# jinlong17/DA-Detect

Hardware: AMD Instinct MI355X
Metric: train images/sec, DA-Faster-RCNN R-50 Cityscapes->Foggy (higher is better)
Workload: dtype f32

## Files before the change

### da_detect_amd/_C.py

```python
import contextlib
import os
import ctypes
import time

import torch

from . import _lib
from . import amax as _amax
from ._lib import ConvDesc

CL = torch.channels_last

NMS_TIE_RULE = 0

PROFILER = None
_KNAME_CACHE = {}


class KernelProfiler(object):

    def __init__(self, pool=0, only=None):
        self.only = only
        self._pool = []
        for _ in range(pool):
# ... 716 lines not shown
        return g_out, g_scaled
    so = ss = None
    if g_out is not None and _amax.slot_of(_amax.carry(g_out, g)) is None:
        so = _amax.new_slot(g.device)
    if scale is not None or _amax.slot_of(_amax.carry(g_scaled, g)) is None:
        ss = _amax.new_slot(g.device)
    _lib.call("dadet_relu_bn_backward_m", _p(g), _p(yy), _p(scale), _p(g_out), _p(g_scaled), rows, C,
              ctypes.c_void_p(so[0]) if so else None, ctypes.c_void_p(ss[0]) if ss else None, _stream())
    if so:
        _amax.attach(g_out, so)
    if ss:
        _amax.attach(g_scaled, ss)
    return g_out, g_scaled


def colsum(g, out=None, accumulate=False, cols=None):
    _dev(g, "g")
    g = _nhwc(g) if g.dim() == 4 else g.contiguous()
    ld = g.shape[1]
    C = ld if cols is None else int(cols)
    rows = g.numel() // ld
    if out is None:
        out = torch.empty(C, dtype=torch.float32, device=g.device)
        accumulate = False
    assert out.numel() == C and out.is_contiguous() and out.dtype == torch.float32
    nbytes = ctypes.c_size_t(0)
    _lib.call("dadet_colsum_workspace_bytes", rows, C, ctypes.byref(nbytes))
    ws = _workspace(nbytes.value, g.device)
    _lib.call("dadet_colsum_ld", _p(g), ld, _p(out), rows, C, 1 if accumulate else 0, _p(ws), ctypes.c_size_t(ws.numel()),
              _stream())
# ... 39 lines not shown
    _dev(x, "x")
    x = _nhwc(x)
    R, C, h, w = x.shape
    y = torch.empty((R, C), dtype=torch.float32, device=x.device)
    _lib.call("dadet_avgpool_forward", _p(x), _p(y), R, h * w, C, _stream())
    return _amax.carry(y, x)


def avgpool_backward(gy, h, w):
    _dev(gy, "gy")
    gy = gy.contiguous()
    R, C = gy.shape
    gx = torch.empty((R, C, h, w), dtype=torch.float32, device=gy.device, memory_format=CL)
    _lib.call("dadet_avgpool_backward", _p(gy), _p(gx), R, h * w, C, _stream())
    return _amax.carry(gx, gy)


def nchw3_to_nhwc4(x):
    _dev(x, "x")
    x = x.contiguous()
    N, C, H, W = x.shape
    assert C == 3
    y = torch.empty((N, 4, H, W), dtype=torch.float32, device=x.device, memory_format=CL)
    _lib.call("dadet_nchw3_to_nhwc4", _p(x), _p(y), N, H, W, _stream())
    if _mode4():
        _amax.ptr(x)
        _amax.carry(y, x)
    return y


# ... 675 lines not shown
```

### da_detect_amd/_lib.py

```python
import ctypes
import os
from ctypes import POINTER, c_char_p, c_float, c_int, c_int64, c_size_t, c_uint64, c_void_p

_HERE = os.path.dirname(os.path.abspath(__file__))
LIB_PATH = os.environ.get("DADET_LIB") or os.path.join(_HERE, "libdadet_hip.so")
_lib = None
DEFAULT_GEMM_MODE = "4"


class ConvDesc(ctypes.Structure):

    _fields_ = [(n, c_int) for n in (
        "N", "H", "W", "Cin", "Cout", "KH", "KW", "stride", "pad", "Ho", "Wo", "OutH", "OutW",
        "out_spatial_stride", "relu_mode")]


class ConvPlanInfo(ctypes.Structure):

    _fields_ = [(n, c_int) for n in (
        "family", "variant", "tiles_m", "tiles_n", "ksplit", "splits", "rows_per_split", "sk_dp_tiles", "sk_tiles", "sk_units",
        "sk_iters", "sk_max_parts", "big_splits", "big_body", "launches", "grid", "needs_counters")] + [
        ("workspace_bytes", c_size_t), ("name", ctypes.c_char * 64)]


# ... 116 lines not shown
    "dadet_sample_anchors": [_P, _P, c_int, c_int, c_int, c_uint64, c_int64, _P, _P, _P, _P, _P],
    "dadet_topk_sorted": [_P, c_int, c_int, c_int64, c_int, _P, _P, _P],
    "dadet_topk_sorted_rows_workspace_bytes": [c_int, c_int, POINTER(c_size_t)],
    "dadet_topk_sorted_rows": [POINTER(TopkRow), c_int, _P, c_size_t, _P],
    "dadet_rpn_anchor_targets": [_P, _P, c_int, _P, c_int, c_float, c_float, _P, _P, _P, _P],
    "dadet_box_match_encode": [_P, c_int, _P, _P, c_int, c_float, c_float, c_float, c_float, c_float, c_float, _P, _P,
                               _P, _P],
    "dadet_roi_pool_forward": [_P, _P, _P, _P, c_int, c_int, c_int, c_int, c_int, c_int, c_int, c_float, _P],
    "dadet_roi_pool_backward": [_P, _P, _P, _P, c_int, c_int, c_int, c_int, c_int, c_int, c_int, _P],
    "dadet_deform_psroi_pool_forward": [_P, _P, _P, _P, _P, c_int, c_int, c_int, c_int, c_int, c_int, c_float,
                                        c_int, c_int, c_int, c_int, c_int, c_float, c_int, _P],
    "dadet_deform_psroi_pool_backward": [_P, _P, _P, _P, _P, _P, _P, c_int, c_int, c_int, c_int, c_int, c_int,
                                         c_float, c_int, c_int, c_int, c_int, c_int, c_float, c_int, _P],
    "dadet_relu_bn_backward": [_P, _P, _P, _P, _P, c_int64, c_int, _P],
    "dadet_relu_bn_backward_m": [_P, _P, _P, _P, _P, c_int64, c_int, _P, _P, _P],
    "dadet_colsum_workspace_bytes": [c_int64, c_int, POINTER(c_size_t)],
    "dadet_colsum": [_P, _P, c_int64, c_int, _P, c_size_t, _P],
    "dadet_colsum_ld": [_P, c_int, _P, c_int64, c_int, c_int, _P, c_size_t, _P],
    "dadet_channel_affine": [_P, _P, _P, _P, c_int64, c_int, c_int, _P],
    "dadet_maxpool3x3s2_forward": [_P, _P, c_int, c_int, c_int, c_int, c_int, c_int, _P],
    "dadet_maxpool3x3s2_relu_backward": [_P, _P, _P, _P, c_int, c_int, c_int, c_int, c_int, c_int, _P, _P],
    "dadet_avgpool_forward": [_P, _P, c_int, c_int, c_int, _P],
    "dadet_avgpool_backward": [_P, _P, c_int, c_int, c_int, _P],
    "dadet_nchw3_to_nhwc4": [_P, _P, c_int, c_int, c_int, _P],
    "dadet_rpn_decode_clip": [_P, _P, _P, c_int, c_float, c_float, c_float, c_float, c_float, c_float, c_float, _P, _P],
    "dadet_da_img_head_loss_forward": [_P, _P, _P, _P, _P, _P, c_int, c_int, c_int, _P],
    "dadet_da_img_head_loss_backward": [_P, _P, _P, _P, _P, _P, _P, _P, _P, c_int, c_int, c_int, _P],
    "dadet_da_img_head_loss_backward_g": [_P, _P, _P, _P, _P, _P, _P, c_float, c_float, _P, _P, _P, _P, c_int, c_int, c_int,
                                          _P],
    "dadet_da_img_head_loss_backward_gm": [_P, _P, _P, _P, _P, _P, _P, c_float, c_float, _P, _P, _P, _P, c_int, c_int, c_int,
                                          _P, _P, _P],
    "dadet_da_ins_tail_forward": [_P, _P, _P, _P, _P, _P, _P, c_int, c_int, c_int, c_int, c_int, _P],
    "dadet_da_ins_tail_backward": [_P, _P, _P, _P, _P, _P, c_float, _P, _P, _P, _P, c_int, c_int, c_int, c_int, c_int, _P],
    "dadet_da_ins_tail_forward_n": [_P, _P, _P, _P, _P, _P, _P, c_int, c_int, POINTER(c_int), c_int, c_int, c_int, _P],
    "dadet_da_ins_tail_backward_n": [_P, _P, _P, _P, _P, _P, c_float, _P, _P, _P, _P, c_int, c_int, POINTER(c_int), c_int,
                                     c_int, c_int, _P],
    "dadet_da_ins_dropout_rows": [_P, _P, _P, c_int64, c_int, _P],
    "dadet_da_ins_merge": [_P, _P, _P, _P, _P, _P, c_int64, c_int, _P],
# ... 45 lines not shown
```

### da_detect_amd/csrc/elementwise.hip

```cpp
#include "box_match.h"
#include "conv_common.h"
#include <float.h>

namespace dadet {

static inline int stream_blocks(int64_t work_items, int threads) {
  int64_t b = ceil_div64(work_items, threads);
  if (b > kMaxStreamBlocks) b = kMaxStreamBlocks;
  if (b < 1) b = 1;
  return (int)b;
}

__global__ void relu_bn_backward_kernel(const float4* __restrict__ g, const float4* __restrict__ y,
                                        const float4* __restrict__ scale, float4* __restrict__ g_out,
                                        float4* __restrict__ g_scaled, int64_t total4, int C4,
                                        unsigned* __restrict__ amax_out, unsigned* __restrict__ amax_scaled) {
  float mo = 0.f, ms = 0.f;
  for (int64_t i = (int64_t)blockIdx.x * blockDim.x + threadIdx.x; i < total4;
       i += (int64_t)gridDim.x * blockDim.x) {
    const float4 gv = g[i];
    float4 r = gv;
    if (y) {
      const float4 yv = y[i];
      r.x = yv.x > 0.f ? gv.x : 0.f;
// ... 3 lines not shown
    }
    if (g_out) g_out[i] = r;
    mo = fmaxf(fmaxf(mo, fmaxf(fabsf(r.x), fabsf(r.y))), fmaxf(fabsf(r.z), fabsf(r.w)));
    if (g_scaled) {
      float4 s = r;
      if (scale) {
        const float4 sc = scale[i % C4];
        s.x *= sc.x; s.y *= sc.y; s.z *= sc.z; s.w *= sc.w;
      }
      g_scaled[i] = s;
      ms = fmaxf(fmaxf(ms, fmaxf(fabsf(s.x), fabsf(s.y))), fmaxf(fabsf(s.z), fabsf(s.w)));
    }
  }
  if (amax_out) amax_publish(amax_out, mo);
  if (amax_scaled) amax_publish(amax_scaled, ms);
}

__global__ __launch_bounds__(256) void colsum_partial_kernel(const float* __restrict__ g,
                                                             float* __restrict__ partial, int64_t rows,
                                                             int C, int64_t rows_per_split, int cb, int ld) {
  __shared__ float red[256];
  const int lanes = 256 / cb;
  const int cl = threadIdx.x % cb, rl = threadIdx.x / cb;
  const int col = blockIdx.x * cb + cl;
  const int64_t r0 = (int64_t)blockIdx.y * rows_per_split;
  int64_t r1 = r0 + rows_per_split;
  if (r1 > rows) r1 = rows;
  float acc = 0.f;
  if (col < C)
    for (int64_t r = r0 + rl; r < r1; r += lanes) acc += g[r * ld + col];
// ... 143 lines not shown
}
__global__ void avgpool_bwd_kernel(const float4* __restrict__ gy, float4* __restrict__ gx, int R, int HW,
                                   int C4) {
  const int64_t total = (int64_t)R * HW * C4;
  const float inv = (float)HW;
  for (int64_t i = (int64_t)blockIdx.x * blockDim.x + threadIdx.x; i < total;
       i += (int64_t)gridDim.x * blockDim.x) {
    const int c = (int)(i % C4);
    const int64_t r = i / ((int64_t)HW * C4);
    float4 g = gy[r * C4 + c];
    g.x /= inv; g.y /= inv; g.z /= inv; g.w /= inv;
    gx[i] = g;
  }
}

__global__ void nchw3_to_nhwc4_kernel(const float* __restrict__ x, float4* __restrict__ y, int N,
                                      int64_t HW) {
  const int64_t total = (int64_t)N * HW;
  for (int64_t i = (int64_t)blockIdx.x * blockDim.x + threadIdx.x; i < total;
       i += (int64_t)gridDim.x * blockDim.x) {
    const int64_t n = i / HW, p = i % HW;
    const float* b = x + n * 3 * HW + p;
    y[i] = make_float4(b[0], b[HW], b[2 * HW], 0.f);
  }
}

__global__ void rpn_decode_clip_kernel(const float4* __restrict__ deltas, const float4* __restrict__ anchors,
                                       const int64_t* __restrict__ topk_idx, int K, float wx, float wy,
                                       float ww, float wh, float xform_clip, float im_w, float im_h,
                                       float4* __restrict__ out) {
// ... 241 lines not shown
  DADET_REQUIRE(rows >= 0 && C > 0 && C % 4 == 0, "relu_bn_backward: C=%d must be a multiple of 4", C);
  if (rows == 0) return DADET_OK;
  DADET_REQUIRE(g && (g_out || g_scaled), "relu_bn_backward: null pointer");
  DADET_REQUIRE(aligned16(g) && aligned16(y) && aligned16(scale) && aligned16(g_out) && aligned16(g_scaled),
                "relu_bn_backward: pointers must be 16-byte aligned");
  const int64_t total4 = rows * (C / 4);
  hipLaunchKernelGGL(relu_bn_backward_kernel, dim3(stream_blocks(total4, 256)), dim3(256), 0,
                     as_stream(stream), reinterpret_cast<const float4*>(g),
                     reinterpret_cast<const float4*>(y), reinterpret_cast<const float4*>(scale),
                     reinterpret_cast<float4*>(g_out), reinterpret_cast<float4*>(g_scaled), total4, C / 4,
                     reinterpret_cast<unsigned*>(g_out ? amax_out : nullptr),
                     reinterpret_cast<unsigned*>(g_scaled ? amax_scaled : nullptr));
  return check_launch("relu_bn_backward");
}

extern "C" int dadet_colsum_workspace_bytes(int64_t rows, int C, size_t* bytes_out) {
  DADET_REQUIRE(rows >= 0 && C > 0 && bytes_out, "colsum_workspace_bytes: bad args");
  *bytes_out = rows == 0 ? 0 : sizeof(float) * (size_t)colsum_splits(rows, C) * C;
  return DADET_OK;
}

extern "C" int dadet_colsum_ld(const float* g, int ld, float* out, int64_t rows, int C, int accumulate, void* workspace,
                               size_t workspace_bytes, void* stream) {
  DADET_REQUIRE(rows >= 0 && C > 0 && ld >= C && out, "colsum: bad args (rows=%lld C=%d ld=%d)", (long long)rows, C, ld);
  hipStream_t st = as_stream(stream);
  if (rows == 0) {
    if (!accumulate) (void)hipMemsetAsync(out, 0, sizeof(float) * C, st);
    return check_launch("colsum(empty)");
  }
  DADET_REQUIRE(g, "colsum: null input");
// ... 65 lines not shown
  if (R == 0) return DADET_OK;
  DADET_REQUIRE(x && y && aligned16(x) && aligned16(y), "avgpool: bad pointers");
  hipLaunchKernelGGL(avgpool_fwd_kernel, dim3(stream_blocks((int64_t)R * (C / 4), 256)), dim3(256), 0,
                     as_stream(stream), reinterpret_cast<const float4*>(x), reinterpret_cast<float4*>(y), R,
                     HW, C / 4);
  return check_launch("avgpool_forward");
}
extern "C" int dadet_avgpool_backward(const float* gy, float* gx, int R, int HW, int C, void* stream) {
  DADET_REQUIRE(R >= 0 && HW > 0 && C > 0 && C % 4 == 0, "avgpool_backward: bad dims");
  if (R == 0) return DADET_OK;
  DADET_REQUIRE(gy && gx && aligned16(gy) && aligned16(gx), "avgpool_backward: bad pointers");
  hipLaunchKernelGGL(avgpool_bwd_kernel, dim3(stream_blocks((int64_t)R * HW * (C / 4), 256)), dim3(256), 0,
                     as_stream(stream), reinterpret_cast<const float4*>(gy), reinterpret_cast<float4*>(gx),
                     R, HW, C / 4);
  return check_launch("avgpool_backward");
}

extern "C" int dadet_nchw3_to_nhwc4(const float* x, float* y, int N, int H, int W, void* stream) {
  DADET_REQUIRE(N >= 0 && H > 0 && W > 0, "nchw3_to_nhwc4: bad dims");
  if (N == 0) return DADET_OK;
  DADET_REQUIRE(x && y && aligned16(y), "nchw3_to_nhwc4: bad pointers");
  const int64_t HW = (int64_t)H * W;
  hipLaunchKernelGGL(nchw3_to_nhwc4_kernel, dim3(stream_blocks((int64_t)N * HW, 256)), dim3(256), 0,
                     as_stream(stream), x, reinterpret_cast<float4*>(y), N, HW);
  return check_launch("nchw3_to_nhwc4");
}

extern "C" int dadet_rpn_decode_clip(const float* deltas, const float* anchors, const int64_t* topk_idx,
                                     int K, float wx, float wy, float ww, float wh, float xform_clip,
                                     float im_w, float im_h, float* boxes_out, void* stream) {
// ... 91 lines not shown
```

### da_detect_amd/csrc/roi_align.hip

```cpp
#include "common.h"

namespace dadet {

struct RoiGeom {
  int batch;
  float start_w, start_h, bin_w, bin_h;
  int grid_h, grid_w;
  float count;
};

__device__ inline RoiGeom roi_geometry(const float* __restrict__ roi, float scale, int pooled_h,
                                       int pooled_w, int sampling_ratio) {
  RoiGeom g;
  g.batch = (int)roi[0];
  g.start_w = roi[1] * scale;
  g.start_h = roi[2] * scale;
  const float end_w = roi[3] * scale;
  const float end_h = roi[4] * scale;
  const float roi_w = fmaxf(end_w - g.start_w, 1.f);
  const float roi_h = fmaxf(end_h - g.start_h, 1.f);
  g.bin_h = roi_h / (float)pooled_h;
  g.bin_w = roi_w / (float)pooled_w;
  g.grid_h = (sampling_ratio > 0) ? sampling_ratio : (int)ceilf(roi_h / (float)pooled_h);
  g.grid_w = (sampling_ratio > 0) ? sampling_ratio : (int)ceilf(roi_w / (float)pooled_w);
// ... 267 lines not shown
          } else {
            acc[0] += q[0] * w / g.count;
          }
        }
      }
    }
    float* dst = grad_in + (size_t)pix * C + c;
    if constexpr (VEC == 4) {
      *reinterpret_cast<float4*>(dst) = make_float4(acc[0], acc[1], acc[2], acc[3]);
    } else {
      dst[0] = acc[0];
    }
  }
}

struct Contribution {
  int row;
  float count;
  float w[4];
  float inv;
  int pow2;
};
constexpr int kListCap = 1024;

__device__ inline int roi_contributions(const RoiGeom& g, int r, int H, int W, int pooled_h, int pooled_w, int y0,
                                        int x0, Contribution* out, int bs = 1) {
  const int out_h = (pooled_h + bs - 1) / bs, out_w = (pooled_w + bs - 1) / bs;
  int sy0, sy1, sx0, sx1, lo, hi, n = 0;
  candidate_range(g.start_h, g.bin_h, g.grid_h, pooled_h, y0, &sy0, &hi);
  candidate_range(g.start_h, g.bin_h, g.grid_h, pooled_h, y0 + 1, &lo, &sy1);
  candidate_range(g.start_w, g.bin_w, g.grid_w, pooled_w, x0, &sx0, &hi);
  candidate_range(g.start_w, g.bin_w, g.grid_w, pooled_w, x0 + 1, &lo, &sx1);
  for (int sy = sy0; sy <= sy1; ++sy) {
    const int ph = sy / g.grid_h, iy = sy - ph * g.grid_h;
    if (bs > 1 && ph % bs) continue;
    const float cy = sample_coord(g.start_h, ph, g.bin_h, iy, g.grid_h);
    const float wy0 = axis_weight(cy, H, y0), wy1 = axis_weight(cy, H, y0 + 1);
    if (wy0 == 0.f && wy1 == 0.f) continue;
    for (int sx = sx0; sx <= sx1; ++sx) {
      const int pw = sx / g.grid_w, ix = sx - pw * g.grid_w;
      if (bs > 1 && pw % bs) continue;
      const float cx = sample_coord(g.start_w, pw, g.bin_w, ix, g.grid_w);
      const float wx0 = axis_weight(cx, W, x0), wx1 = axis_weight(cx, W, x0 + 1);
      if (wx0 == 0.f && wx1 == 0.f) continue;
      if (out) {
        Contribution c;
        c.row = (r * out_h + ph / bs) * out_w + pw / bs;
        c.count = g.count;
        c.w[0] = wy0 * wx0; c.w[1] = wy0 * wx1; c.w[2] = wy1 * wx0; c.w[3] = wy1 * wx1;
        c.inv = 1.f / g.count;
        const int ci = (int)g.count;
        c.pow2 = (ci & (ci - 1)) == 0;
        out[n] = c;
      }
      ++n;
    }
  }
  return n;
}

template <int VEC, int MAXC>
__global__ __launch_bounds__(256) void roi_align_bwd_list_kernel(
    const float* __restrict__ grad_out, const float* __restrict__ rois, float* __restrict__ grad_in, int B, int C,
    int H, int W, int R, int pooled_h, int pooled_w, float scale, int sampling_ratio, int bin_stride,
    const int64_t* __restrict__ levels, int level) {
  __shared__ Contribution s_list[kListCap];
  __shared__ int s_ids[256];
  __shared__ int s_wave_n[4];
  __shared__ int s_total;
  const int tiles_x = (W + 1) / 2, tiles_y = (H + 1) / 2;
  const int sx = (tiles_x + 1) / 2, sy = (tiles_y + 1) / 2;
  const int xcd = blockIdx.x % kNumXCD, idx = blockIdx.x / kNumXCD;
  const int super = (idx >> 2) * kNumXCD + xcd, q = idx & 3;
  const int b = super / (sx * sy);
  const int ty = ((super / sx) % sy) * 2 + (q >> 1), tx = (super % sx) * 2 + (q & 1);
  if (b >= B || ty >= tiles_y || tx >= tiles_x) return;
  const int y0 = ty * 2;
  const int x0 = tx * 2;
  const int lane = threadIdx.x & 63, wave = threadIdx.x >> 6;
  float acc[MAXC][4][VEC];
#pragma unroll
  for (int k = 0; k < MAXC; ++k)
#pragma unroll
    for (int p = 0; p < 4; ++p)
#pragma unroll
      for (int v = 0; v < VEC; ++v) acc[k][p][v] = 0.f;

  auto accumulate = [&](int n_entries) {
    constexpr int U = MAXC == 1 ? 8 : 4;
#pragma unroll 1
    for (int e0 = 0; e0 < n_entries; e0 += U) {
#pragma unroll
      for (int k = 0; k < MAXC; ++k) {
        const int c = (threadIdx.x + k * 256) * VEC;
        if (c >= C) break;
        float gq[U][VEC];
#pragma unroll
        for (int u = 0; u < U; ++u) {
          const int e = min(e0 + u, n_entries - 1);
          const float* src = grad_out + (size_t)s_list[e].row * C + c;
          if constexpr (VEC == 4) {
            const float4 t = *reinterpret_cast<const float4*>(src);
            gq[u][0] = t.x; gq[u][1] = t.y; gq[u][2] = t.z; gq[u][3] = t.w;
          } else {
            gq[u][0] = src[0];
          }
        }
#pragma unroll
        for (int u = 0; u < U; ++u) {
          if (e0 + u >= n_entries) break;
          const Contribution q = s_list[e0 + u];
#pragma unroll
          for (int p = 0; p < 4; ++p) {
            if (q.w[p] == 0.f) continue;
#pragma unroll
            for (int v = 0; v < VEC; ++v) {
              const float t = gq[u][v] * q.w[p];
              acc[k][p][v] += q.pow2 ? t * q.inv : t / q.count;
            }
          }
        }
      }
    }
  };

  for (int base = 0; base < R; base += 256) {
    const int r = base + (int)threadIdx.x;
    bool hit = false;
    if (r < R) {
      const RoiGeom g = roi_geometry(rois + (size_t)r * 5, scale, pooled_h, pooled_w, sampling_ratio);
      hit = g.batch == b && (!levels || levels[r] == (int64_t)level) && roi_touches_tile(g, pooled_h, pooled_w, y0, x0);
    }
    const unsigned long long ballot = __ballot(hit);
    if (lane == 0) s_wave_n[wave] = __popcll(ballot);
    __syncthreads();
    int before = 0;
    for (int wv = 0; wv < wave; ++wv) before += s_wave_n[wv];
    const int ntouch = s_wave_n[0] + s_wave_n[1] + s_wave_n[2] + s_wave_n[3];
    if (hit) s_ids[before + __popcll(ballot & ((1ULL << lane) - 1ULL))] = r;
    __syncthreads();
    for (int start = 0; start < ntouch; start += 64) {
      const int nround = min(64, ntouch - start);
      if (wave == 0) {
        int my_n = 0, rr = -1;
        RoiGeom g;
        if (lane < nround) {
          rr = s_ids[start + lane];
          g = roi_geometry(rois + (size_t)rr * 5, scale, pooled_h, pooled_w, sampling_ratio);
          my_n = roi_contributions(g, rr, H, W, pooled_h, pooled_w, y0, x0, nullptr, bin_stride);
        }
        int incl = my_n;
#pragma unroll
        for (int off = 1; off < 64; off <<= 1) {
          const int t = __shfl_up(incl, off, 64);
          if (lane >= off) incl += t;
        }
        const int total = __shfl(incl, 63, 64);
        if (lane == 0) s_total = total;
        if (total <= kListCap && rr >= 0)
          roi_contributions(g, rr, H, W, pooled_h, pooled_w, y0, x0, s_list + (incl - my_n), bin_stride);
      }
      __syncthreads();
      const int total = s_total;
      if (total <= kListCap) {
        accumulate(total);
      } else {
        for (int i = 0; i < nround; ++i) {
          __syncthreads();
          if (threadIdx.x == 0) {
            const int r1 = s_ids[start + i];
            const RoiGeom g1 = roi_geometry(rois + (size_t)r1 * 5, scale, pooled_h, pooled_w, sampling_ratio);
            const int n1 = roi_contributions(g1, r1, H, W, pooled_h, pooled_w, y0, x0, nullptr, bin_stride);
            if (n1 <= kListCap) roi_contributions(g1, r1, H, W, pooled_h, pooled_w, y0, x0, s_list, bin_stride);
            s_total = n1 <= kListCap ? n1 : -1;
          }
          __syncthreads();
          if (s_total < 0) __builtin_trap();
          accumulate(s_total);
        }
      }
      __syncthreads();
    }
  }
#pragma unroll
  for (int p = 0; p < 4; ++p) {
    const int y = y0 + (p >> 1), x = x0 + (p & 1);
    if (y >= H || x >= W) continue;
#pragma unroll
    for (int k = 0; k < MAXC; ++k) {
      const int c = (threadIdx.x + k * 256) * VEC;
      if (c >= C) break;
      float* dst = grad_in + ((size_t)(b * H + y) * W + x) * C + c;
      if constexpr (VEC == 4) {
        *reinterpret_cast<float4*>(dst) = make_float4(acc[k][p][0], acc[k][p][1], acc[k][p][2], acc[k][p][3]);
// ... 179 lines not shown
```

### da_detect_amd/layers/misc.py

```python

import torch
from torch import nn
from torch.autograd import Function
from torch.autograd.function import once_differentiable

from .. import _C
from .. import amax as _amax
from .conv import conv2d_affine_act

CL = torch.channels_last


class FrozenBatchNorm2d(nn.Module):

    def __init__(self, n):
        super(FrozenBatchNorm2d, self).__init__()
        self.register_buffer("weight", torch.ones(n))
        self.register_buffer("bias", torch.zeros(n))
        self.register_buffer("running_mean", torch.zeros(n))
        self.register_buffer("running_var", torch.ones(n))
        self._cache = None

    def folded(self):
        key = (self.weight._version, self.bias._version, self.running_mean._version,
# ... 265 lines not shown


class SigmoidFocalLoss(nn.Module):

    def __init__(self, gamma, alpha):
        super(SigmoidFocalLoss, self).__init__()
        self.gamma, self.alpha = gamma, alpha

    def forward(self, logits, targets):
        return sigmoid_focal_loss(logits, targets, self.gamma, self.alpha).sum()

    def __repr__(self):
        return "{}(gamma={}, alpha={})".format(self.__class__.__name__, self.gamma, self.alpha)


class _AvgPoolHW(Function):

    @staticmethod
    def forward(ctx, x):
        ctx.hw = (x.shape[2], x.shape[3])
        return _C.avgpool_forward(x)

    @staticmethod
    @once_differentiable
    def backward(ctx, g):
        return _C.avgpool_backward(g, *ctx.hw)


_POOL_MEMO = True


def global_avg_pool(x):
    if x.shape[0] == 0:
        return x.new_empty((0, x.shape[1]))
    memo = x.__dict__.get("_dadet_pooled") if _POOL_MEMO else None
    if memo is not None and memo[0] == x._version and memo[1] == torch.is_grad_enabled():
        return memo[2]
    y = _AvgPoolHW.apply(x)
    x._dadet_pooled = (x._version, torch.is_grad_enabled(), y)
    return y
# ... 1 lines not shown
```

### da_detect_amd/modeling/backbone/resnet.py

```python
from collections import namedtuple

import torch
import torch.nn.functional as F
from torch import nn

from ... import _C
from ...layers import Conv2d, FrozenBatchNorm2d, conv2d_affine_act
from ...utils.registry import Registry
from ...utils import streams
from ...utils.streams import WgradLane

StageSpec = namedtuple("StageSpec", ["index", "block_count", "return_features"])


def _specs(*rows):
    return tuple(StageSpec(index=i, block_count=c, return_features=r) for (i, c, r) in rows)


ResNet50StagesTo5 = _specs((1, 3, False), (2, 4, False), (3, 6, False), (4, 3, True))
ResNet50StagesTo4 = _specs((1, 3, False), (2, 4, False), (3, 6, True))
ResNet101StagesTo5 = _specs((1, 3, False), (2, 4, False), (3, 23, False), (4, 3, True))
ResNet101StagesTo4 = _specs((1, 3, False), (2, 4, False), (3, 23, True))
ResNet50FPNStagesTo5 = _specs((1, 3, True), (2, 4, True), (3, 6, True), (4, 3, True))
ResNet101FPNStagesTo5 = _specs((1, 3, True), (2, 4, True), (3, 23, True), (4, 3, True))
ResNet152FPNStagesTo5 = _specs((1, 3, True), (2, 8, True), (3, 36, True), (4, 3, True))


_WGRAD_BATCH = True
_WGRAD_GROUP = __import__("os").environ.get("DADET_WGRAD_GROUP", "1") == "1"


class _WgradGroup(object):

    _known = {}

    def __init__(self, lane, batch, weights):
        self.lane, self.batch, self.reqs = lane, batch, []
        self.on = (_WGRAD_GROUP and batch is not None and _C._mode4() and 2 <= len(weights) <= _C.WGRAD_GROUP_MAX
                   and all(streams.direct_grad_target(w) is not None for w in weights))
        self.key = None
        if self.on:
            self.key = tuple(tuple(w.shape) for w in weights) + (lane.on,)
            self.on = self._known.get(self.key, True) is not False

# ... 18 lines not shown
                    _C.conv_wgrad(r["x"], r["gy"], r["weight_shape"], r["stride"], r["pad"], out_scale=r["out_scale"],
                                  dw=r["dw"], accumulate=True, pending=batch)

        self.lane.run_group(run, *[t for r in reqs for t in (r["x"], r["gy"])])
        self.reqs = []


class _BlockBackward(object):

    def __init__(self, needs, x, w1, wd, s1, sd, stride):
        self.need_x, self.n1, self.n2, self.n3, nd = needs
        self.nd = nd and wd is not None
        self.x, self.w1, self.wd, self.s1, self.sd, self.stride = x, w1, wd, s1, sd, stride

    def open(self, G, out, out_private, y2, w2, w3, s3):
        self.S3 = G.contiguous(memory_format=torch.channels_last) if out_private else _C.relu_bn_backward(G, out, None)[1]
        self.lane = WgradLane(G.device, rows=G.shape[0] * G.shape[2] * G.shape[3])
        self.batch = _C.WgradBatch() if _WGRAD_BATCH else None
        weights = ((w3, self.n3), (w2, self.n2), (self.w1, self.n1), (self.wd, self.nd))
        self.group = _WgradGroup(self.lane, self.batch, [w for w, need in weights if need])
        dw3 = self.wgrad(w3, y2, self.S3, 1, 0, s3) if self.n3 else None
        return _C.conv_forward(self.S3, _C.conv_weight_transpose(w3, s3), relu_mode=2, mask_ref=y2), dw3

    def wgrad(self, w, xin, gout, st, pd, sc, shape=None, grouped=True):
        shape = tuple(w.shape) if shape is None else shape
        batch = self.batch
        if grouped and self.group.take(w, xin, gout, st, pd, sc, shape=shape):
            return None
        return self.lane.run_into(w, lambda acc: _C.conv_wgrad(xin, gout, shape, st, pd, out_scale=sc, dw=acc,
                                                               accumulate=True, pending=batch),
                                  lambda: _C.conv_wgrad(xin, gout, shape, st, pd, out_scale=sc, pending=batch),
# ... 326 lines not shown
def _make_stage(block, in_channels, bottleneck_channels, out_channels, block_count, num_groups,
                stride_in_1x1, first_stride, dilation=1, dcn_config=None):
    blocks, stride = [], first_stride
    for _ in range(block_count):
        blocks.append(block(in_channels, bottleneck_channels, out_channels, num_groups, stride_in_1x1, stride,
                            dilation=dilation, dcn_config=dcn_config))
        stride = 1
        in_channels = out_channels
    return _Stage(*blocks)


class _Stage(nn.Sequential):

    input_is_relu = False

    def forward(self, x, first_stride=None):
        n = len(self)
        blocks = list(self)
        for i, block in enumerate(blocks):
            private = i < n - 1 and blocks[i + 1].uses_fused_path()
            if i == 0 and first_stride is not None:
                x = block(x, in_relu=self.input_is_relu, out_private=private, stride=first_stride)
            else:
                x = block(x, in_relu=(i > 0 or self.input_is_relu), out_private=private)
        return x


class ResNet(nn.Module):
    def __init__(self, cfg):
        super(ResNet, self).__init__()
        stem_module = _STEM_MODULES[cfg.MODEL.RESNETS.STEM_FUNC]
        stage_specs = _STAGE_SPECS[cfg.MODEL.BACKBONE.CONV_BODY]
        block = _TRANSFORMATION_MODULES[cfg.MODEL.RESNETS.TRANS_FUNC]
        self.stem = stem_module(cfg)
        num_groups = cfg.MODEL.RESNETS.NUM_GROUPS
# ... 4 lines not shown
        for spec in stage_specs:
            name = "layer" + str(spec.index)
            factor = 2 ** (spec.index - 1)
            out_channels = stage2_out * factor
            self.add_module(name, _make_stage(block, in_channels, stage2_bottleneck * factor, out_channels,
                                              spec.block_count, num_groups, cfg.MODEL.RESNETS.STRIDE_IN_1X1,
                                              first_stride=int(spec.index > 1) + 1,
                                              dcn_config={
                                                  "stage_with_dcn": cfg.MODEL.RESNETS.STAGE_WITH_DCN[spec.index - 1],
                                                  "with_modulated_dcn": cfg.MODEL.RESNETS.WITH_MODULATED_DCN,
                                                  "deformable_groups": cfg.MODEL.RESNETS.DEFORMABLE_GROUPS}))
            in_channels = out_channels
            getattr(self, name).input_is_relu = spec.index > 1
            self.stages.append(name)
            self.return_features[name] = spec.return_features
        self._freeze_backbone(cfg.MODEL.BACKBONE.FREEZE_CONV_BODY_AT)

    def _freeze_backbone(self, freeze_at):
        for stage_index in range(max(freeze_at, 0)):
            m = self.stem if stage_index == 0 else getattr(self, "layer" + str(stage_index))
            for p in m.parameters():
                p.requires_grad = False

    def forward(self, x):
        outputs = []
        x = self.stem(x)
        for name in self.stages:
            x = getattr(self, name)(x)
            if self.return_features[name]:
                outputs.append(x)
        return outputs


class ResNetHead(nn.Module):

    def __init__(self, block_module, stages, num_groups=1, width_per_group=64, stride_in_1x1=True,
                 stride_init=None, res2_out_channels=256, dilation=1):
        super(ResNetHead, self).__init__()
        factor = 2 ** (stages[0].index - 1)
        out_channels = res2_out_channels * factor
        in_channels = out_channels // 2
        bottleneck_channels = num_groups * width_per_group * factor
        block = _TRANSFORMATION_MODULES[block_module]
# ... 32 lines not shown
```

### include/dadet.h

```cpp
#ifndef DADET_H_
#define DADET_H_

#include <stddef.h>
#include <stdint.h>

#ifdef __cplusplus
extern "C" {
#endif

#define DADET_OK 0
#define DADET_EINVAL (-1)
#define DADET_ELAUNCH (-2)
#define DADET_EWORKSPACE (-3)
#define DADET_EUNSUPPORTED (-4)

const char* dadet_last_error(void);
int dadet_version(void);
int dadet_device_info(int* cu_count, int* clock_khz, size_t* hbm_bytes, char* arch_name, int arch_name_len);

int dadet_nms_workspace_bytes(int n, size_t* bytes_out);
int dadet_nms(const float* boxes_xyxy, const float* scores, int n, float thresh, int tie_rule,
              int max_keep, void* workspace, size_t workspace_bytes, int64_t* keep_out,
              int* num_keep_out, void* stream);
int dadet_nms_batch_workspace_bytes(int batch, int n_max, size_t* bytes_out);
// ... 261 lines not shown
int dadet_deform_psroi_pool_forward(const float* data, const float* rois, const float* trans, float* out,
                                    float* top_count, int B, int H, int W, int C, int R, int no_trans,
                                    float spatial_scale, int output_dim, int group_size, int pooled_size,
                                    int part_size, int sample_per_part, float trans_std, int num_classes,
                                    void* stream);
int dadet_deform_psroi_pool_backward(const float* grad_out, const float* top_count, const float* data,
                                     const float* rois, const float* trans, float* grad_data, float* grad_trans,
                                     int B, int H, int W, int C, int R, int no_trans, float spatial_scale,
                                     int output_dim, int group_size, int pooled_size, int part_size,
                                     int sample_per_part, float trans_std, int num_classes, void* stream);

int dadet_relu_bn_backward(const float* g, const float* y, const float* scale, float* g_out,
                           float* g_scaled, int64_t rows, int C, void* stream);
int dadet_relu_bn_backward_m(const float* g, const float* y, const float* scale, float* g_out, float* g_scaled,
                             int64_t rows, int C, float* amax_out, float* amax_scaled, void* stream);
int dadet_colsum_workspace_bytes(int64_t rows, int C, size_t* bytes_out);
int dadet_colsum_ld(const float* g, int ld, float* out, int64_t rows, int C, int accumulate, void* workspace,
                    size_t workspace_bytes, void* stream);
int dadet_colsum(const float* g, float* out, int64_t rows, int C, void* workspace, size_t workspace_bytes,
                 void* stream);
int dadet_channel_affine(const float* x, const float* scale, const float* bias, float* y, int64_t rows,
                         int C, int relu, void* stream);
int dadet_maxpool3x3s2_forward(const float* x, float* y, int N, int H, int W, int C, int Ho, int Wo,
                               void* stream);
int dadet_maxpool3x3s2_relu_backward(const float* y, const float* gp, const float* scale, float* g, int N, int H,
                                     int W, int C, int Ho, int Wo, float* amax_out, void* stream);
int dadet_avgpool_forward(const float* x, float* y, int R, int HW, int C, void* stream);
int dadet_avgpool_backward(const float* gy, float* gx, int R, int HW, int C, void* stream);
int dadet_nchw3_to_nhwc4(const float* x, float* y, int N, int H, int W, void* stream);

int dadet_rpn_decode_clip(const float* deltas, const float* anchors, const int64_t* topk_idx, int K,
                          float wx, float wy, float ww, float wh, float xform_clip, float im_w,
                          float im_h, float* boxes_out, void* stream);

int dadet_da_img_head_loss_forward(const float* t, const float* w2, const float* b2, const float* labels,
                                   float* logits_out, float* sums_out, int num_images,
                                   int rows_per_image, int C1, void* stream);
int dadet_da_img_head_loss_backward(const float* t, const float* w2, const float* logits,
                                    const float* labels, const float* coef, float* g_t_w, float* g_t_x,
                                    float* g_w2, float* g_b2, int num_images, int rows_per_image, int C1,
                                    void* stream);
int dadet_da_img_head_loss_backward_g(const float* t, const float* w2, const float* logits, const float* labels,
                                      const float* g_bce, const float* g_mean_sig, const float* w_adv_dev, float w_adv,
// ... 44 lines not shown
```

Before: 162.0.

## Broadcast avgpool grad into ReLU backward, regroup ROIAlign backward lists, private stage outputs

Avgpool backward now produces a stride-0 broadcast view, and the ROI head's ResNet block detects it and runs a fused ReLU-mask kernel that reads the pooled gradient directly. This skips materialising the full spatial gradient tensor. ROIAlign backward's shared-memory contribution list is restructured into groups of rows with per-term weights, so each distinct grad_out row is loaded once into a register ring and reused, cutting redundant global loads. Separately, backbone stage outputs are marked private when the next stage uses the fused path, and a wave-occupancy hint is added. These add complexity and rely on tensor-version and stride checks for the broadcast path to be correct.

```diff
diff --git a/da_detect_amd/_C.py b/da_detect_amd/_C.py
--- a/da_detect_amd/_C.py
+++ b/da_detect_amd/_C.py
@@ -754,6 +754,22 @@
     return g_out, g_scaled
 
 
+def relu_bn_backward_bcast(g, y):
+    _dev(g, "g"), _dev(y, "y")
+    g, y = g.contiguous(), _nhwc(y)
+    R, C, h, w = y.shape
+    assert tuple(g.shape) == (R, C), "relu_bn_backward_bcast: g %s for y %s" % (tuple(g.shape), tuple(y.shape))
+    out = torch.empty_like(y)
+    slot = None
+    if _mode4() and _amax.slot_of(_amax.carry(out, g)) is None:
+        slot = _amax.new_slot(g.device)
+    _lib.call("dadet_relu_bn_backward_bcast_m", _p(g), _p(y), _p(out), R, h * w, C,
+              ctypes.c_void_p(slot[0]) if slot else None, _stream())
+    if slot:
+        _amax.attach(out, slot)
+    return out
+
+
 def colsum(g, out=None, accumulate=False, cols=None):
     _dev(g, "g")
     g = _nhwc(g) if g.dim() == 4 else g.contiguous()
@@ -823,6 +839,25 @@
     gx = torch.empty((R, C, h, w), dtype=torch.float32, device=gy.device, memory_format=CL)
     _lib.call("dadet_avgpool_backward", _p(gy), _p(gx), R, h * w, C, _stream())
     return _amax.carry(gx, gy)
+
+
+def avgpool_backward_broadcast(gy, h, w):
+    _dev(gy, "gy")
+    gy = gy.contiguous()
+    R, C = gy.shape
+    q = torch.empty_like(gy)
+    _lib.call("dadet_avgpool_backward_rows", _p(gy), _p(q), R, h * w, C, _stream())
+    gx = q.view(R, C, 1, 1).expand(R, C, h, w)
+    gx._dadet_pool_grad = (gy, gy._version)
+    return _amax.carry(gx, gy)
+
+
+def pool_grad_source(G):
+    src = G.__dict__.get("_dadet_pool_grad")
+    if src is None or src[0]._version != src[1] or G.dim() != 4 or \
+            (G.shape[2] * G.shape[3] > 1 and (G.stride(2) != 0 or G.stride(3) != 0)):
+        return None
+    return src[0]
 
 
 def nchw3_to_nhwc4(x):
diff --git a/da_detect_amd/_lib.py b/da_detect_amd/_lib.py
--- a/da_detect_amd/_lib.py
+++ b/da_detect_amd/_lib.py
@@ -154,6 +154,7 @@
                                          c_float, c_int, c_int, c_int, c_int, c_int, c_float, c_int, _P],
     "dadet_relu_bn_backward": [_P, _P, _P, _P, _P, c_int64, c_int, _P],
     "dadet_relu_bn_backward_m": [_P, _P, _P, _P, _P, c_int64, c_int, _P, _P, _P],
+    "dadet_relu_bn_backward_bcast_m": [_P, _P, _P, c_int, c_int, c_int, _P, _P],
     "dadet_colsum_workspace_bytes": [c_int64, c_int, POINTER(c_size_t)],
     "dadet_colsum": [_P, _P, c_int64, c_int, _P, c_size_t, _P],
     "dadet_colsum_ld": [_P, c_int, _P, c_int64, c_int, c_int, _P, c_size_t, _P],
@@ -162,6 +163,7 @@
     "dadet_maxpool3x3s2_relu_backward": [_P, _P, _P, _P, c_int, c_int, c_int, c_int, c_int, c_int, _P, _P],
     "dadet_avgpool_forward": [_P, _P, c_int, c_int, c_int, _P],
     "dadet_avgpool_backward": [_P, _P, c_int, c_int, c_int, _P],
+    "dadet_avgpool_backward_rows": [_P, _P, c_int, c_int, c_int, _P],
     "dadet_nchw3_to_nhwc4": [_P, _P, c_int, c_int, c_int, _P],
     "dadet_rpn_decode_clip": [_P, _P, _P, c_int, c_float, c_float, c_float, c_float, c_float, c_float, c_float, _P, _P],
     "dadet_da_img_head_loss_forward": [_P, _P, _P, _P, _P, _P, c_int, c_int, c_int, _P],
diff --git a/da_detect_amd/csrc/elementwise.hip b/da_detect_amd/csrc/elementwise.hip
--- a/da_detect_amd/csrc/elementwise.hip
+++ b/da_detect_amd/csrc/elementwise.hip
@@ -41,6 +41,29 @@
   }
   if (amax_out) amax_publish(amax_out, mo);
   if (amax_scaled) amax_publish(amax_scaled, ms);
+}
+
+__global__ void relu_bcast_backward_kernel(const float4* __restrict__ g, const float4* __restrict__ y,
+                                           float4* __restrict__ out, int64_t total4, int HW, int C4,
+                                           unsigned* __restrict__ amax_out) {
+  float mo = 0.f;
+  const float div = (float)HW;
+  for (int64_t i = (int64_t)blockIdx.x * blockDim.x + threadIdx.x; i < total4;
+       i += (int64_t)gridDim.x * blockDim.x) {
+    const int c = (int)(i % C4);
+    const int64_t r = i / ((int64_t)HW * C4);
+    float4 q = g[r * C4 + c];
+    q.x /= div; q.y /= div; q.z /= div; q.w /= div;
+    const float4 yv = y[i];
+    float4 o;
+    o.x = yv.x > 0.f ? q.x : 0.f;
+    o.y = yv.y > 0.f ? q.y : 0.f;
+    o.z = yv.z > 0.f ? q.z : 0.f;
+    o.w = yv.w > 0.f ? q.w : 0.f;
+    out[i] = o;
+    mo = fmaxf(fmaxf(mo, fmaxf(fabsf(o.x), fabsf(o.y))), fmaxf(fabsf(o.z), fabsf(o.w)));
+  }
+  if (amax_out) amax_publish(amax_out, mo);
 }
 
 __global__ __launch_bounds__(256) void colsum_partial_kernel(const float* __restrict__ g,
@@ -214,6 +237,16 @@
   }
 }
 
+__global__ void avgpool_bwd_rows_kernel(const float4* __restrict__ gy, float4* __restrict__ q, int64_t total4, int HW) {
+  const float inv = (float)HW;
+  for (int64_t i = (int64_t)blockIdx.x * blockDim.x + threadIdx.x; i < total4;
+       i += (int64_t)gridDim.x * blockDim.x) {
+    float4 g = gy[i];
+    g.x /= inv; g.y /= inv; g.z /= inv; g.w /= inv;
+    q[i] = g;
+  }
+}
+
 __global__ void nchw3_to_nhwc4_kernel(const float* __restrict__ x, float4* __restrict__ y, int N,
                                       int64_t HW) {
   const int64_t total = (int64_t)N * HW;
@@ -485,6 +518,19 @@
   return check_launch("relu_bn_backward");
 }
 
+extern "C" int dadet_relu_bn_backward_bcast_m(const float* g, const float* y, float* g_out, int R, int HW, int C,
+                                              float* amax_out, void* stream) {
+  DADET_REQUIRE(R >= 0 && HW > 0 && C > 0 && C % 4 == 0, "relu_bn_backward_bcast: bad dims R=%d HW=%d C=%d", R, HW, C);
+  if (R == 0) return DADET_OK;
+  DADET_REQUIRE(g && y && g_out, "relu_bn_backward_bcast: null pointer");
+  DADET_REQUIRE(aligned16(g) && aligned16(y) && aligned16(g_out), "relu_bn_backward_bcast: pointers must be 16-byte aligned");
+  const int64_t total4 = (int64_t)R * HW * (C / 4);
+  hipLaunchKernelGGL(relu_bcast_backward_kernel, dim3(stream_blocks(total4, 256)), dim3(256), 0, as_stream(stream),
+                     reinterpret_cast<const float4*>(g), reinterpret_cast<const float4*>(y),
+                     reinterpret_cast<float4*>(g_out), total4, HW, C / 4, reinterpret_cast<unsigned*>(amax_out));
+  return check_launch("relu_bn_backward_bcast");
+}
+
 extern "C" int dadet_colsum_workspace_bytes(int64_t rows, int C, size_t* bytes_out) {
   DADET_REQUIRE(rows >= 0 && C > 0 && bytes_out, "colsum_workspace_bytes: bad args");
   *bytes_out = rows == 0 ? 0 : sizeof(float) * (size_t)colsum_splits(rows, C) * C;
@@ -580,6 +626,16 @@
                      as_stream(stream), reinterpret_cast<const float4*>(gy), reinterpret_cast<float4*>(gx),
                      R, HW, C / 4);
   return check_launch("avgpool_backward");
+}
+
+extern "C" int dadet_avgpool_backward_rows(const float* gy, float* q, int R, int HW, int C, void* stream) {
+  DADET_REQUIRE(R >= 0 && HW > 0 && C > 0 && C % 4 == 0, "avgpool_backward_rows: bad dims");
+  if (R == 0) return DADET_OK;
+  DADET_REQUIRE(gy && q && aligned16(gy) && aligned16(q), "avgpool_backward_rows: bad pointers");
+  const int64_t total4 = (int64_t)R * (C / 4);
+  hipLaunchKernelGGL(avgpool_bwd_rows_kernel, dim3(stream_blocks(total4, 256)), dim3(256), 0, as_stream(stream),
+                     reinterpret_cast<const float4*>(gy), reinterpret_cast<float4*>(q), total4, HW);
+  return check_launch("avgpool_backward_rows");
 }
 
 extern "C" int dadet_nchw3_to_nhwc4(const float* x, float* y, int N, int H, int W, void* stream) {
diff --git a/da_detect_amd/csrc/roi_align.hip b/da_detect_amd/csrc/roi_align.hip
--- a/da_detect_amd/csrc/roi_align.hip
+++ b/da_detect_amd/csrc/roi_align.hip
@@ -305,57 +305,95 @@
   }
 }
 
-struct Contribution {
-  int row;
+struct GroupHdr {
+  int row0;
+  int term0;
   float count;
-  float w[4];
-  float inv;
-  int pow2;
 };
-constexpr int kListCap = 1024;
-
-__device__ inline int roi_contributions(const RoiGeom& g, int r, int H, int W, int pooled_h, int pooled_w, int y0,
-                                        int x0, Contribution* out, int bs = 1) {
+struct RoiList { int terms, groups, rows; };
+constexpr int kTermCap = 1024;
+constexpr int kGroupCap = 512;
+constexpr int kRowCap = 1024;
+
+__device__ inline RoiList roi_contributions(const RoiGeom& g, int r, int H, int W, int pooled_h, int pooled_w, int y0,
+                                            int x0, int bs, RoiList at, float4* s_w, unsigned char* s_slot, int* s_rows,
+                                            GroupHdr* s_groups) {
   const int out_h = (pooled_h + bs - 1) / bs, out_w = (pooled_w + bs - 1) / bs;
-  int sy0, sy1, sx0, sx1, lo, hi, n = 0;
+  int sy0, sy1, sx0, sx1, lo, hi;
   candidate_range(g.start_h, g.bin_h, g.grid_h, pooled_h, y0, &sy0, &hi);
   candidate_range(g.start_h, g.bin_h, g.grid_h, pooled_h, y0 + 1, &lo, &sy1);
   candidate_range(g.start_w, g.bin_w, g.grid_w, pooled_w, x0, &sx0, &hi);
   candidate_range(g.start_w, g.bin_w, g.grid_w, pooled_w, x0 + 1, &lo, &sx1);
+  int nx = 0, npw = 0, last_pw = -1;
+  for (int sx = sx0; sx <= sx1; ++sx) {
+    const int pw = sx / g.grid_w, ix = sx - pw * g.grid_w;
+    if (bs > 1 && pw % bs) continue;
+    const float cx = sample_coord(g.start_w, pw, g.bin_w, ix, g.grid_w);
+    if (axis_weight(cx, W, x0) == 0.f && axis_weight(cx, W, x0 + 1) == 0.f) continue;
+    ++nx;
+    if (pw != last_pw) { ++npw; last_pw = pw; }
+  }
+  RoiList n = {0, 0, 0};
+  if (nx == 0) return n;
+  int cur_ph = -1;
   for (int sy = sy0; sy <= sy1; ++sy) {
     const int ph = sy / g.grid_h, iy = sy - ph * g.grid_h;
     if (bs > 1 && ph % bs) continue;
     const float cy = sample_coord(g.start_h, ph, g.bin_h, iy, g.grid_h);
     const float wy0 = axis_weight(cy, H, y0), wy1 = axis_weight(cy, H, y0 + 1);
     if (wy0 == 0.f && wy1 == 0.f) continue;
-    for (int sx = sx0; sx <= sx1; ++sx) {
-      const int pw = sx / g.grid_w, ix = sx - pw * g.grid_w;
-      if (bs > 1 && pw % bs) continue;
-      const float cx = sample_coord(g.start_w, pw, g.bin_w, ix, g.grid_w);
-      const float wx0 = axis_weight(cx, W, x0), wx1 = axis_weight(cx, W, x0 + 1);
-      if (wx0 == 0.f && wx1 == 0.f) continue;
-      if (out) {
-        Contribution c;
-        c.row = (r * out_h + ph / bs) * out_w + pw / bs;
-        c.count = g.count;
-        c.w[0] = wy0 * wx0; c.w[1] = wy0 * wx1; c.w[2] = wy1 * wx0; c.w[3] = wy1 * wx1;
-        c.inv = 1.f / g.count;
-        const int ci = (int)g.count;
-        c.pow2 = (ci & (ci - 1)) == 0;
-        out[n] = c;
-      }
-      ++n;
+    const bool new_group = ph != cur_ph;
+    if (new_group) {
+      cur_ph = ph;
+      if (s_w) {
+        GroupHdr h;
+        h.row0 = at.rows + n.rows;
+        h.term0 = at.terms + n.terms;
+        h.count = g.count;
+        s_groups[at.groups + n.groups] = h;
+      }
+    }
+    if (s_w) {
+      int slot = -1;
+      last_pw = -1;
+      for (int sx = sx0; sx <= sx1; ++sx) {
+        const int pw = sx / g.grid_w, ix = sx - pw * g.grid_w;
+        if (bs > 1 && pw % bs) continue;
+        const float cx = sample_coord(g.start_w, pw, g.bin_w, ix, g.grid_w);
+        const float wx0 = axis_weight(cx, W, x0), wx1 = axis_weight(cx, W, x0 + 1);
+        if (wx0 == 0.f && wx1 == 0.f) continue;
+        if (pw != last_pw) {
+          ++slot;
+          last_pw = pw;
+          if (new_group) s_rows[at.rows + n.rows + slot] = (r * out_h + ph / bs) * out_w + pw / bs;
+        }
+        s_w[at.terms + n.terms] = make_float4(wy0 * wx0, wy0 * wx1, wy1 * wx0, wy1 * wx1);
+        s_slot[at.terms + n.terms] = (unsigned char)slot;
+        ++n.terms;
+      }
+    } else {
+      n.terms += nx;
+    }
+    if (new_group) {
+      ++n.groups;
+      n.rows += npw;
     }
   }
   return n;
 }
 
+__device__ inline int uniform(int v) { return __builtin_amdgcn_readfirstlane(v); }
+__device__ inline float uniform(float v) { return __int_as_float(__builtin_amdgcn_readfirstlane(__float_as_int(v))); }
+
 template <int VEC, int MAXC>
-__global__ __launch_bounds__(256) void roi_align_bwd_list_kernel(
+__global__ __launch_bounds__(256) __attribute__((amdgpu_waves_per_eu(MAXC == 1 ? 4 : 2))) void roi_align_bwd_list_kernel(
     const float* __restrict__ grad_out, const float* __restrict__ rois, float* __restrict__ grad_in, int B, int C,
     int H, int W, int R, int pooled_h, int pooled_w, float scale, int sampling_ratio, int bin_stride,
     const int64_t* __restrict__ levels, int level) {
-  __shared__ Contribution s_list[kListCap];
+  __shared__ float4 s_w[kTermCap];
+  __shared__ unsigned char s_slot[kTermCap];
+  __shared__ int s_rows[kRowCap];
+  __shared__ GroupHdr s_groups[kGroupCap + 1];
   __shared__ int s_ids[256];
   __shared__ int s_wave_n[4];
   __shared__ int s_total;
@@ -377,41 +415,117 @@
 #pragma unroll
       for (int v = 0; v < VEC; ++v) acc[k][p][v] = 0.f;
 
-  auto accumulate = [&](int n_entries) {
+  auto apply = [&](float (&a)[4][VEC], const float (&gv)[VEC], const float (&w)[4], float count, float inv, bool pow2) {
+    if (pow2) {
+#pragma unroll
+      for (int p = 0; p < 4; ++p) {
+        if (w[p] == 0.f) continue;
+#pragma unroll
+        for (int v = 0; v < VEC; ++v) a[p][v] += (gv[v] * w[p]) * inv;
+      }
+    } else {
+#pragma unroll
+      for (int p = 0; p < 4; ++p) {
+        if (w[p] == 0.f) continue;
+#pragma unroll
+        for (int v = 0; v < VEC; ++v) a[p][v] += (gv[v] * w[p]) / count;
+      }
+    }
+  };
+  auto load_row = [&](float (&dst)[VEC], int row, int c) {
+    const float* src = grad_out + (size_t)row * C + c;
+    if constexpr (VEC == 4) {
+      const float4 t = *reinterpret_cast<const float4*>(src);
+      dst[0] = t.x; dst[1] = t.y; dst[2] = t.z; dst[3] = t.w;
+    } else {
+      dst[0] = src[0];
+    }
+  };
+  auto lane_i = [](int v, int l) { return __builtin_amdgcn_readlane(v, l); };
+  auto lane_f = [](float v, int l) { return __int_as_float(__builtin_amdgcn_readlane(__float_as_int(v), l)); };
+
+  const int wave_c0 = uniform((int)(threadIdx.x >> 6)) * 64 * VEC;
+  auto accumulate = [&](int n_groups) {
     constexpr int U = MAXC == 1 ? 8 : 4;
+    int gi = 0;
 #pragma unroll 1
-    for (int e0 = 0; e0 < n_entries; e0 += U) {
+    while (gi < n_groups) {
+      const int hl = min(gi + lane, n_groups);
+      const int h_row0 = s_groups[hl].row0, h_term0 = s_groups[hl].term0;
+      const float h_count = s_groups[hl].count;
+      const int row_a = lane_i(h_row0, 0);
+      const unsigned long long over = __ballot(h_row0 - row_a > U);
+      int m = min((over ? (int)__builtin_ctzll(over) : 64) - 1, n_groups - gi);
+      m = uniform(m < 1 ? 1 : m);
+      const int nrows = lane_i(h_row0, m) - row_a;
+      const int term_a = lane_i(h_term0, 0), term_e = lane_i(h_term0, m);
 #pragma unroll
       for (int k = 0; k < MAXC; ++k) {
-        const int c = (threadIdx.x + k * 256) * VEC;
-        if (c >= C) break;
-        float gq[U][VEC];
-#pragma unroll
-        for (int u = 0; u < U; ++u) {
-          const int e = min(e0 + u, n_entries - 1);
-          const float* src = grad_out + (size_t)s_list[e].row * C + c;
-          if constexpr (VEC == 4) {
-            const float4 t = *reinterpret_cast<const float4*>(src);
-            gq[u][0] = t.x; gq[u][1] = t.y; gq[u][2] = t.z; gq[u][3] = t.w;
-          } else {
-            gq[u][0] = src[0];
+        if (wave_c0 + k * 256 * VEC >= C) break;
+        const int c = min(((int)threadIdx.x + k * 256) * VEC, C - VEC);
+        typedef float Ring __attribute__((ext_vector_type(U * VEC)));
+        Ring ring;
+        float gq[VEC];
+        if (nrows <= U) {
+#pragma unroll
+          for (int u = 0; u < U; ++u) {
+            load_row(gq, s_rows[row_a + min(u, nrows - 1)], c);
+#pragma unroll
+            for (int v = 0; v < VEC; ++v) ring[u * VEC + v] = gq[v];
           }
-        }
-#pragma unroll
-        for (int u = 0; u < U; ++u) {
-          if (e0 + u >= n_entries) break;
-          const Contribution q = s_list[e0 + u];
-#pragma unroll
-          for (int p = 0; p < 4; ++p) {
-            if (q.w[p] == 0.f) continue;
-#pragma unroll
-            for (int v = 0; v < VEC; ++v) {
-              const float t = gq[u][v] * q.w[p];
-              acc[k][p][v] += q.pow2 ? t * q.inv : t / q.count;
+          int tb = term_a;
+          int tl = min(tb + lane, kTermCap - 1);
+          int v_slot = s_slot[tl];
+          float4 v_w = s_w[tl];
+#pragma unroll 1
+          for (int j = 0; j < m; ++j) {
+            const int off = lane_i(h_row0, j) - row_a;
+            const int t0 = lane_i(h_term0, j), t1 = lane_i(h_term0, j + 1);
+            const float count = lane_f(h_count, j), inv = 1.f / count;
+            const int ci = (int)count;
+            const bool pow2 = (ci & (ci - 1)) == 0;
+#pragma unroll 1
+            for (int t = t0; t < t1; ++t) {
+              if (t - tb >= 64) {
+                tb = t;
+                tl = min(tb + lane, kTermCap - 1);
+                v_slot = s_slot[tl];
+                v_w = s_w[tl];
+              }
+              const int i = t - tb;
+              const int slot = off + lane_i(v_slot, i);
+              const float w[4] = {lane_f(v_w.x, i), lane_f(v_w.y, i), lane_f(v_w.z, i), lane_f(v_w.w, i)};
+              float gv[VEC];
+#pragma unroll
+              for (int v = 0; v < VEC; ++v) gv[v] = ring[slot * VEC + v];
+              apply(acc[k], gv, w, count, inv, pow2);
             }
           }
-        }
-      }
+        } else {
+          const float count = lane_f(h_count, 0), inv = 1.f / count;
+          const int ci = (int)count;
+          const bool pow2 = (ci & (ci - 1)) == 0;
+#pragma unroll 1
+          for (int e0 = term_a; e0 < term_e; e0 += U) {
+#pragma unroll
+            for (int u = 0; u < U; ++u) {
+              load_row(gq, s_rows[row_a + s_slot[min(e0 + u, term_e - 1)]], c);
+#pragma unroll
+              for (int v = 0; v < VEC; ++v) ring[u * VEC + v] = gq[v];
+            }
+#pragma unroll
+            for (int u = 0; u < U; ++u) {
+              if (e0 + u >= term_e) break;
+              const float4 wq = s_w[e0 + u];
+              const float w[4] = {uniform(wq.x), uniform(wq.y), uniform(wq.z), uniform(wq.w)};
+#pragma unroll
+              for (int v = 0; v < VEC; ++v) gq[v] = ring[u * VEC + v];
+              apply(acc[k], gq, w, count, inv, pow2);
+            }
+          }
+        }
+      }
+      gi += m;
     }
   };
 
@@ -433,42 +547,67 @@
     for (int start = 0; start < ntouch; start += 64) {
       const int nround = min(64, ntouch - start);
       if (wave == 0) {
-        int my_n = 0, rr = -1;
+        RoiList mine = {0, 0, 0};
+        int rr = -1;
         RoiGeom g;
         if (lane < nround) {
           rr = s_ids[start + lane];
           g = roi_geometry(rois + (size_t)rr * 5, scale, pooled_h, pooled_w, sampling_ratio);
-          my_n = roi_contributions(g, rr, H, W, pooled_h, pooled_w, y0, x0, nullptr, bin_stride);
-        }
-        int incl = my_n;
+          mine = roi_contributions(g, rr, H, W, pooled_h, pooled_w, y0, x0, bin_stride, mine, nullptr, nullptr, nullptr,
+                                   nullptr);
+        }
+        RoiList incl = mine;
 #pragma unroll
         for (int off = 1; off < 64; off <<= 1) {
-          const int t = __shfl_up(incl, off, 64);
-          if (lane >= off) incl += t;
-        }
-        const int total = __shfl(incl, 63, 64);
-        if (lane == 0) s_total = total;
-        if (total <= kListCap && rr >= 0)
-          roi_contributions(g, rr, H, W, pooled_h, pooled_w, y0, x0, s_list + (incl - my_n), bin_stride);
+          const int t = __shfl_up(incl.terms, off, 64), gr = __shfl_up(incl.groups, off, 64);
+          const int rw = __shfl_up(incl.rows, off, 64);
+          if (lane >= off) { incl.terms += t; incl.groups += gr; incl.rows += rw; }
+        }
+        RoiList total;
+        total.terms = __shfl(incl.terms, 63, 64);
+        total.groups = __shfl(incl.groups, 63, 64);
+        total.rows = __shfl(incl.rows, 63, 64);
+        const bool fits = total.terms <= kTermCap && total.groups <= kGroupCap && total.rows <= kRowCap;
+        if (lane == 0) {
+          s_total = fits ? total.groups : -1;
+          if (fits) {
+            GroupHdr end;
+            end.row0 = total.rows; end.term0 = total.terms; end.count = 1.f;
+            s_groups[total.groups] = end;
+          }
+        }
+        if (fits && rr >= 0) {
+          RoiList at;
+          at.terms = incl.terms - mine.terms; at.groups = incl.groups - mine.groups; at.rows = incl.rows - mine.rows;
+          roi_contributions(g, rr, H, W, pooled_h, pooled_w, y0, x0, bin_stride, at, s_w, s_slot, s_rows, s_groups);
+        }
       }
       __syncthreads();
       const int total = s_total;
-      if (total <= kListCap) {
-        accumulate(total);
-      } else {
-        for (int i = 0; i < nround; ++i) {
+      const int passes = total >= 0 ? 1 : nround;
+#pragma unroll 1
+      for (int i = 0; i < passes; ++i) {
+        if (total < 0) {
           __syncthreads();
           if (threadIdx.x == 0) {
             const int r1 = s_ids[start + i];
             const RoiGeom g1 = roi_geometry(rois + (size_t)r1 * 5, scale, pooled_h, pooled_w, sampling_ratio);
-            const int n1 = roi_contributions(g1, r1, H, W, pooled_h, pooled_w, y0, x0, nullptr, bin_stride);
-            if (n1 <= kListCap) roi_contributions(g1, r1, H, W, pooled_h, pooled_w, y0, x0, s_list, bin_stride);
-            s_total = n1 <= kListCap ? n1 : -1;
+            const RoiList at = {0, 0, 0};
+            const RoiList n1 = roi_contributions(g1, r1, H, W, pooled_h, pooled_w, y0, x0, bin_stride, at, nullptr,
+                                                 nullptr, nullptr, nullptr);
+            const bool fits = n1.terms <= kTermCap && n1.groups <= kGroupCap && n1.rows <= kRowCap;
+            if (fits) {
+              roi_contributions(g1, r1, H, W, pooled_h, pooled_w, y0, x0, bin_stride, at, s_w, s_slot, s_rows, s_groups);
+              GroupHdr end;
+              end.row0 = n1.rows; end.term0 = n1.terms; end.count = 1.f;
+              s_groups[n1.groups] = end;
+            }
+            s_total = fits ? n1.groups : -1;
           }
           __syncthreads();
           if (s_total < 0) __builtin_trap();
-          accumulate(s_total);
-        }
+        }
+        accumulate(total >= 0 ? total : s_total);
       }
       __syncthreads();
     }
diff --git a/da_detect_amd/layers/misc.py b/da_detect_amd/layers/misc.py
--- a/da_detect_amd/layers/misc.py
+++ b/da_detect_amd/layers/misc.py
@@ -303,6 +303,9 @@
         return "{}(gamma={}, alpha={})".format(self.__class__.__name__, self.gamma, self.alpha)
 
 
+_POOL_GRAD_VIEW = True
+
+
 class _AvgPoolHW(Function):
 
     @staticmethod
@@ -313,6 +316,8 @@
     @staticmethod
     @once_differentiable
     def backward(ctx, g):
+        if _POOL_GRAD_VIEW:
+            return _C.avgpool_backward_broadcast(g, *ctx.hw)
         return _C.avgpool_backward(g, *ctx.hw)
 
 
diff --git a/da_detect_amd/modeling/backbone/resnet.py b/da_detect_amd/modeling/backbone/resnet.py
--- a/da_detect_amd/modeling/backbone/resnet.py
+++ b/da_detect_amd/modeling/backbone/resnet.py
@@ -28,6 +28,7 @@
 
 _WGRAD_BATCH = True
 _WGRAD_GROUP = __import__("os").environ.get("DADET_WGRAD_GROUP", "1") == "1"
+_STAGE_PRIVATE = True
 
 
 class _WgradGroup(object):
@@ -76,7 +77,13 @@
         self.x, self.w1, self.wd, self.s1, self.sd, self.stride = x, w1, wd, s1, sd, stride
 
     def open(self, G, out, out_private, y2, w2, w3, s3):
-        self.S3 = G.contiguous(memory_format=torch.channels_last) if out_private else _C.relu_bn_backward(G, out, None)[1]
+        pooled = None if out_private else _C.pool_grad_source(G)
+        if out_private:
+            self.S3 = G.contiguous(memory_format=torch.channels_last)
+        elif pooled is not None:
+            self.S3 = _C.relu_bn_backward_bcast(pooled, out)
+        else:
+            self.S3 = _C.relu_bn_backward(G, out, None)[1]
         self.lane = WgradLane(G.device, rows=G.shape[0] * G.shape[2] * G.shape[3])
         self.batch = _C.WgradBatch() if _WGRAD_BATCH else None
         weights = ((w3, self.n3), (w2, self.n2), (self.w1, self.n1), (self.wd, self.nd))
@@ -433,11 +440,14 @@
 
     input_is_relu = False
 
-    def forward(self, x, first_stride=None):
+    def forward(self, x, first_stride=None, out_private=False):
         n = len(self)
         blocks = list(self)
         for i, block in enumerate(blocks):
-            private = i < n - 1 and blocks[i + 1].uses_fused_path()
+            if i < n - 1:
+                private = blocks[i + 1].uses_fused_path()
+            else:
+                private = out_private
             if i == 0 and first_stride is not None:
                 x = block(x, in_relu=self.input_is_relu, out_private=private, stride=first_stride)
             else:
@@ -472,7 +482,14 @@
             getattr(self, name).input_is_relu = spec.index > 1
             self.stages.append(name)
             self.return_features[name] = spec.return_features
+        self.private_output = {name: False for name in self.stages}
+        for name, nxt in zip(self.stages, self.stages[1:]):
+            self.private_output[name] = self._stage_output_private(name, nxt)
         self._freeze_backbone(cfg.MODEL.BACKBONE.FREEZE_CONV_BODY_AT)
+
+    def _stage_output_private(self, name, nxt):
+        nxt = getattr(self, nxt)
+        return (not self.return_features[name]) and nxt.input_is_relu and nxt[0].uses_fused_path()
 
     def _freeze_backbone(self, freeze_at):
         for stage_index in range(max(freeze_at, 0)):
@@ -484,7 +501,7 @@
         outputs = []
         x = self.stem(x)
         for name in self.stages:
-            x = getattr(self, name)(x)
+            x = getattr(self, name)(x, out_private=_STAGE_PRIVATE and self.private_output[name])
             if self.return_features[name]:
                 outputs.append(x)
         return outputs
diff --git a/include/dadet.h b/include/dadet.h
--- a/include/dadet.h
+++ b/include/dadet.h
@@ -299,6 +299,8 @@
                            float* g_scaled, int64_t rows, int C, void* stream);
 int dadet_relu_bn_backward_m(const float* g, const float* y, const float* scale, float* g_out, float* g_scaled,
                              int64_t rows, int C, float* amax_out, float* amax_scaled, void* stream);
+int dadet_relu_bn_backward_bcast_m(const float* g, const float* y, float* g_out, int R, int HW, int C, float* amax_out,
+                                   void* stream);
 int dadet_colsum_workspace_bytes(int64_t rows, int C, size_t* bytes_out);
 int dadet_colsum_ld(const float* g, int ld, float* out, int64_t rows, int C, int accumulate, void* workspace,
                     size_t workspace_bytes, void* stream);
@@ -312,6 +314,7 @@
                                      int W, int C, int Ho, int Wo, float* amax_out, void* stream);
 int dadet_avgpool_forward(const float* x, float* y, int R, int HW, int C, void* stream);
 int dadet_avgpool_backward(const float* gy, float* gx, int R, int HW, int C, void* stream);
+int dadet_avgpool_backward_rows(const float* gy, float* q, int R, int HW, int C, void* stream);
 int dadet_nchw3_to_nhwc4(const float* x, float* y, int N, int H, int W, void* stream);
 
 int dadet_rpn_decode_clip(const float* deltas, const float* anchors, const int64_t* topk_idx, int K,
```

Result: faster. 163.7, median of 6 (+1.1%).
